# dwipddalal/AttWarp

Measured on AMD Instinct MI355X. Metric: warped images/sec, higher is better.
Workload: dtype f32

## Files before the change

attwarp_amd/csrc/attn_f32v.hpp:

```cpp
#pragma once
#include <type_traits>
#include "common.hpp"

namespace attwarp {

constexpr int ATTN_NT = 256;

struct SharedDiv {
  float d, r1;
  __device__ __forceinline__ explicit SharedDiv(float den) : d(den) {
    const float r0 = __builtin_amdgcn_rcpf(den);
    const float e0 = __builtin_fmaf(-den, r0, 1.0f);
    r1 = __builtin_fmaf(e0, r0, r0);
  }
  __device__ __forceinline__ float operator()(float a) const {
    const float q0 = fmul(a, r1);
    const float e1 = __builtin_fmaf(-d, q0, a);
    const float q1 = __builtin_fmaf(e1, r1, q0);
    const float e2 = __builtin_fmaf(-d, q1, a);
    return __builtin_fmaf(e2, r1, q1);
  }
  __device__ __forceinline__ float first_refinement(float a) const {
    const float q0 = fmul(a, r1);
    const float e1 = __builtin_fmaf(-d, q0, a);
// ... 44 lines not shown
template <typename T> struct Raw4 { uint32_t lo, hi; };
template <> struct Raw4<float> { float x, y, z, w; };
template <typename T> __device__ __forceinline__ Raw4<T> load4_raw(const T* p) {
  typedef uint16_t v4h_a2 __attribute__((ext_vector_type(4), aligned(2)));
  const v4h_a2 q = __builtin_nontemporal_load(reinterpret_cast<const v4h_a2*>(p));
  return Raw4<T>{(uint32_t)q.x | ((uint32_t)q.y << 16), (uint32_t)q.z | ((uint32_t)q.w << 16)};
}
template <> __device__ __forceinline__ Raw4<float> load4_raw<float>(const float* p) {
  const F4v q = load4_nt<float>(p);
  return Raw4<float>{q.x, q.y, q.z, q.w};
}
__device__ __forceinline__ F4v cvt4(const Raw4<float>& r) { return F4v{r.x, r.y, r.z, r.w}; }
__device__ __forceinline__ F4v cvt4(const Raw4<__half>& r) {
  return F4v{__half2float(__builtin_bit_cast(__half, (uint16_t)(r.lo & 0xffffu))), __half2float(__builtin_bit_cast(__half, (uint16_t)(r.lo >> 16))),
             __half2float(__builtin_bit_cast(__half, (uint16_t)(r.hi & 0xffffu))), __half2float(__builtin_bit_cast(__half, (uint16_t)(r.hi >> 16)))};
}
__device__ __forceinline__ F4v cvt4(const Raw4<__hip_bfloat16>& r) {
  return F4v{__uint_as_float(r.lo << 16), __uint_as_float(r.lo & 0xffff0000u), __uint_as_float(r.hi << 16),
             __uint_as_float(r.hi & 0xffff0000u)};
}
template <typename T> __device__ __forceinline__ float round_to(float v) { return to_f32<T>(from_f32<T>(v)); }
template <> __device__ __forceinline__ float round_to<float>(float v) { return v; }

template <typename T>
struct AttnStepArgsT {
  const T* attn;
  int heads;
  int64_t sb, sh, row_off;
  const int32_t* starts;
  int starts_mod, max_start, ntok;
  T* out;
};
typedef AttnStepArgsT<float> AttnStepArgs;
struct AttnStepArgsAny {
  const void* attn;
  int dtype;
  int heads;
  int64_t sb, sh, row_off;
  const int32_t* starts;
  int starts_mod, max_start, ntok;
  void* out;
  template <typename T>
  __device__ __forceinline__ AttnStepArgsT<T> as() const {
    AttnStepArgsT<T> a;
    a.attn = static_cast<const T*>(attn); a.heads = heads; a.sb = sb; a.sh = sh; a.row_off = row_off; a.starts = starts;
    a.starts_mod = starts_mod; a.max_start = max_start; a.ntok = ntok; a.out = static_cast<T*>(out);
    return a;
  }
};
template <int NV>
constexpr size_t attn_v4_lds_bytes() { return (size_t)(ATTN_NT / WAVE) * NV * 4 * WAVE * sizeof(float); }

template <typename T, int NV, int HU>
__device__ __forceinline__ void attn_reduce_v4_block(const AttnStepArgsT<T>& a, int b, float* part) {
  constexpr int NT = ATTN_NT, PW = NV * 4 * WAVE, NW = NT / WAVE;
  const int heads = a.heads, ntok = a.ntok;
  const int64_t sh = a.sh;
  const int lane = threadIdx.x & (WAVE - 1), wid = __builtin_amdgcn_readfirstlane(threadIdx.x / WAVE);
  const int st = min(max(a.starts[b % a.starts_mod], 0), a.max_start);
  const T* base = a.attn + (int64_t)b * a.sb + a.row_off + st;
  float acc[NV][4];
#pragma unroll
  for (int i = 0; i < NV; ++i) acc[i][0] = acc[i][1] = acc[i][2] = acc[i][3] = 0.0f;

  auto head_ptr = [&](int h) { return base + (int64_t)min(h, heads - 1) * sh; };
  const bool tail_room = st + 3 <= a.max_start && ntok < NV * 4 * WAVE;
  auto misalign = [&](const T* rp) { return tail_room ? (int)((reinterpret_cast<uintptr_t>(rp) / sizeof(T)) & 1u) : 0; };
  constexpr bool ALIGN16 = sizeof(T) == 2;
  auto load = [&](Raw4<T> (&r)[HU][NV], int h0) {
#pragma unroll
    for (int u = 0; u < HU; ++u) {
      const T* rp = head_ptr(h0 + u * NW);
      if constexpr (ALIGN16) {
        const int mis = misalign(rp);
        const T* ap = rp - mis;
        const int cmax = (mis + ntok - 1) >> 2;
#pragma unroll
        for (int i = 0; i < NV; ++i) {
          unsigned bo = (unsigned)min(lane + WAVE * i, cmax) * 4u * (unsigned)sizeof(T);
          asm volatile("" : "+v"(bo));
          typedef uint32_t v2u __attribute__((ext_vector_type(2), aligned(2)));
          const v2u q = __builtin_nontemporal_load(reinterpret_cast<const v2u*>(reinterpret_cast<const char*>(ap) + bo));
          r[u][i].lo = q.x;
          r[u][i].hi = q.y;
        }
      } else {
#pragma unroll
        for (int i = 0; i < NV; ++i) {
          const int t = min(4 * lane + 4 * WAVE * i, ntok - 4);
          unsigned bo = (unsigned)t * (unsigned)sizeof(T);
          asm volatile("" : "+v"(bo));
          r[u][i] = load4_raw<T>(reinterpret_cast<const T*>(reinterpret_cast<const char*>(rp) + bo));
        }
      }
    }
  };
  auto next_dword = [&](uint32_t own, uint32_t next_vec) -> uint32_t {
    const uint32_t rot = __builtin_amdgcn_update_dpp(0u, next_vec, 0x134, 0xf, 0xf, false);
    return __builtin_amdgcn_update_dpp(rot, own, 0x130, 0xf, 0xf, false);
  };
  auto realign = [&](const Raw4<T> (&r)[NV], int mis, Raw4<T> (&o)[NV]) {
    if (!ALIGN16 || mis == 0) {
#pragma unroll
      for (int i = 0; i < NV; ++i) o[i] = r[i];
      return;
    }
    if constexpr (ALIGN16) {
#pragma unroll
      for (int i = 0; i < NV; ++i) {
        const Raw4<T>& n = r[i + 1 < NV ? i + 1 : i];
        const uint32_t w2 = next_dword(r[i].lo, n.lo);
        o[i].lo = __builtin_amdgcn_alignbyte(r[i].hi, r[i].lo, 2);
        o[i].hi = __builtin_amdgcn_alignbyte(w2, r[i].hi, 2);
      }
    }
  };
  auto reduce = [&](const Raw4<T> (&r)[HU][NV], int h0) {
#pragma unroll
    for (int u = 0; u < HU; ++u) {
      if (h0 + u * NW < heads) {
        F4v v[NV];
        Raw4<T> sh4[NV];
        realign(r[u], misalign(head_ptr(h0 + u * NW)), sh4);
#pragma unroll
        for (int i = 0; i < NV; ++i) v[i] = cvt4(sh4[i]);
        float s = 0.0f;
#pragma unroll
        for (int i = 0; i < NV; ++i)
          if (4 * lane + 4 * WAVE * i < ntok)
            s = fadd(s, fadd(fadd(v[i].x, v[i].y), fadd(v[i].z, v[i].w)));
        s = wave_sum_dpp(s);
        const float den = to_f32<T>(add_tiny<T>(from_f32<T>(s)));
        constexpr bool kNeedLo = !std::is_same<T, __half>::value;
        uint32_t lo = 0xffffffffu, hi = 0u;
#pragma unroll
        for (int i = 0; i < NV; ++i) {
          const uint32_t bx = __float_as_uint(v[i].x), by = __float_as_uint(v[i].y),
                         bz = __float_as_uint(v[i].z), bw = __float_as_uint(v[i].w);
          if (kNeedLo) lo = min(min(lo, bx - 1u), min(by - 1u, min(bz - 1u, bw - 1u)));
          hi = max(max(hi, bx), max(by, max(bz, bw)));
        }
        const bool box = den >= 8.673617379884035e-19f && den <= 4.0f &&
                         __all(lo >= SDIV_NUM_LO - 1u && hi <= SDIV_NUM_HI);
        if (box) {
          const SharedDiv dv(den);
#pragma unroll
          for (int i = 0; i < NV; ++i) {
            acc[i][0] = fadd(acc[i][0], dv.template rounded_to<T>(v[i].x));
            acc[i][1] = fadd(acc[i][1], dv.template rounded_to<T>(v[i].y));
            acc[i][2] = fadd(acc[i][2], dv.template rounded_to<T>(v[i].z));
            acc[i][3] = fadd(acc[i][3], dv.template rounded_to<T>(v[i].w));
          }
        } else {
#pragma unroll
          for (int i = 0; i < NV; ++i) {
            acc[i][0] = fadd(acc[i][0], round_to<T>(v[i].x / den));
            acc[i][1] = fadd(acc[i][1], round_to<T>(v[i].y / den));
            acc[i][2] = fadd(acc[i][2], round_to<T>(v[i].z / den));
            acc[i][3] = fadd(acc[i][3], round_to<T>(v[i].w / den));
          }
        }
      }
    }
  };
  constexpr int HS = NW * HU;
  for (int h0 = wid; h0 < heads; h0 += HS) {
    Raw4<T> r[HU][NV];
    load(r, h0);
    reduce(r, h0);
  }
#pragma unroll
  for (int i = 0; i < NV; ++i)
#pragma unroll
    for (int j = 0; j < 4; ++j) part[wid * PW + 4 * lane + 4 * WAVE * i + j] = acc[i][j];
  __syncthreads();
  const float nheads = to_f32<T>(from_f32<T>((float)heads));
  for (int t = threadIdx.x; t < ntok; t += NT) {
    float m = 0.0f;
#pragma unroll
    for (int w = 0; w < NW; ++w) m = fadd(m, part[w * PW + t]);
    a.out[(int64_t)b * ntok + t] = from_f32<T>(round_to<T>(m) / nheads);
  }
}


}
```

attwarp_amd/csrc/attn_maps.hip:

```cpp
#include "common.hpp"
#include "axis_blocks.hpp"
#include "attn_f32v.hpp"

#include <algorithm>
#include <cstring>

namespace attwarp {

template <typename T>
__global__ __launch_bounds__(ATTN_NT, 5) void attn_maps_kernel(const AttnStepArgsT<T> a, const StepsMapsArgs m, int n_maps8) {
  extern __shared__ __attribute__((aligned(16))) float am_smem[];
  __shared__ float s_tmp[64], s_pm[64];
  const int blk = blockIdx.x;
  if (blk < n_maps8) {
    if (blk < 2 * m.B) axis_maps_from_steps_block<8, T>(m, blk >> 1, blk & 1, reinterpret_cast<double*>(am_smem), s_tmp, s_pm);
    return;
  }
  attn_reduce_v4_block<T, 3, 4>(a, blk - n_maps8, am_smem);
}

template <typename T>
static int launch_attn_maps(const void* rows, int n_rows, int heads, int kv_len, const int32_t* starts, int starts_mod,
                            int ntok, void* steps_out, const StepsMapsArgs& m, hipStream_t st) {
  AttnStepArgsT<T> a;
  a.attn = static_cast<const T*>(rows); a.heads = heads; a.sb = (int64_t)heads * kv_len; a.sh = kv_len; a.row_off = 0;
  a.starts = starts; a.starts_mod = starts_mod; a.max_start = kv_len - ntok; a.ntok = ntok; a.out = static_cast<T*>(steps_out);
  const int n_maps8 = ((2 * m.B + 7) / 8) * 8;
  const size_t lds = std::max(attn_v4_lds_bytes<3>(), steps_maps_lds_bytes(std::max(m.W, m.H), m.g));
  if (const int rc = grant_dynamic_lds(attn_maps_kernel<T>, lds, "attn_reduce_and_maps")) return rc;
  hipLaunchKernelGGL((attn_maps_kernel<T>), dim3(n_maps8 + n_rows), dim3(ATTN_NT), lds, st, a, m, n_maps8);
  return check_launch("attn_maps_kernel");
}

}

using namespace attwarp;

extern "C" int attwarp_attn_reduce_and_maps(int attn_dtype, const void* rows, int n_rows, int heads, int kv_len,
                                            const int32_t* starts, int starts_mod, int ntok, void* steps_out,
                                            const void* steps_in, int T, int B, int g, int W, int H, int W_out, int H_out,
                                            const double* inv_x, const double* inv_y, float* map_x, float* map_y,
                                            void* stream) {
  ATTWARP_REQUIRE(rows && starts && steps_out && steps_in && inv_x && inv_y && map_x && map_y,
                  "attn_reduce_and_maps: null pointer");
  ATTWARP_REQUIRE(n_rows > 0 && heads > 0 && kv_len > 0 && ntok > 0 && starts_mod > 0 && T > 0 && B > 0 && g > 0 && W > 0 &&
                  H > 0 && W_out > 0 && H_out > 0, "attn_reduce_and_maps: non-positive size");
  ATTWARP_REQUIRE(attn_dtype == ATTWARP_F32 || attn_dtype == ATTWARP_F16 || attn_dtype == ATTWARP_BF16,
                  "attn_reduce_and_maps: attn_dtype must be F32, F16 or BF16 (got %d)", attn_dtype);
  ATTWARP_REQUIRE(ntok <= kv_len, "attn_reduce_and_maps: ntok=%d > kv_len=%d", ntok, kv_len);
  ATTWARP_REQUIRE(steps_out != steps_in, "attn_reduce_and_maps: steps_out must not alias steps_in");
  if (ntok % 4 != 0 || ntok > 3 * 4 * WAVE || ntok != g * g)
    return fail(ATTWARP_E_UNSUPPORTED, "attn_reduce_and_maps: ntok must equal g*g, be a multiple of 4 and <= 768");
  if (g > 32 || std::max(W, H) > 8192 || B > 65535)
    return fail(ATTWARP_E_UNSUPPORTED, "attn_reduce_and_maps: g > 32, max(W,H) > 8192 or B > 65535");
  StepsMapsArgs m;
  m.steps = steps_in; m.step_dtype = attn_dtype; m.T = T; m.B = B; m.g = g; m.W = W; m.H = H; m.W_out = W_out; m.H_out = H_out;
  m.inv_x = inv_x; m.inv_y = inv_y; m.map_x = map_x; m.map_y = map_y; m.att_out = nullptr;
  hipStream_t st = as_stream(stream);
  if (attn_dtype == ATTWARP_F32) return launch_attn_maps<float>(rows, n_rows, heads, kv_len, starts, starts_mod, ntok, steps_out, m, st);
  if (attn_dtype == ATTWARP_F16) return launch_attn_maps<__half>(rows, n_rows, heads, kv_len, starts, starts_mod, ntok, steps_out, m, st);
  return launch_attn_maps<__hip_bfloat16>(rows, n_rows, heads, kv_len, starts, starts_mod, ntok, steps_out, m, st);
}
```

attwarp_amd/csrc/common.hpp:

```cpp
#pragma once
#include <hip/hip_runtime.h>
#include <hip/hip_fp16.h>
#include <hip/hip_bf16.h>
#include <cstdarg>
#include <cstdint>
#include <cstdio>

#include "../../include/attwarp.h"

namespace attwarp {

constexpr int WAVE = 64;

char* error_buffer();
int fail(int code, const char* fmt, ...);

#define ATTWARP_REQUIRE(cond, ...)                                   \
  do {                                                               \
    if (!(cond)) return ::attwarp::fail(ATTWARP_E_ARG, __VA_ARGS__); \
  } while (0)

inline int check_launch(const char* what) {
  hipError_t e = hipGetLastError();
  if (e != hipSuccess) return fail(ATTWARP_E_LAUNCH, "%s: %s", what, hipGetErrorString(e));
  return ATTWARP_OK;
}

__device__ __forceinline__ float fmul(float a, float b) { return __fmul_rn(a, b); }
__device__ __forceinline__ float fadd(float a, float b) { return __fadd_rn(a, b); }
__device__ __forceinline__ float fsub(float a, float b) { return __fsub_rn(a, b); }
__device__ __forceinline__ int cv_round_q5(float m) {
  const float s = fmul(m, 32.0f);
  return (s >= -2147483648.0f && s < 2147483648.0f) ? __float2int_rn(s) : (int)0x80000000;
}
__device__ __forceinline__ float clamp_coord(float m, int size) { return fminf(fmaxf(m, -1.0f), (float)size); }
__device__ __forceinline__ float lerp_rn(float a, float b, float t) { return fadd(a, fmul(t, fsub(b, a))); }

template <typename T>
__device__ __forceinline__ T wave_sum(T v) {
#pragma unroll
  for (int o = WAVE / 2; o > 0; o >>= 1) v += __shfl_xor(v, o, WAVE);
  return v;
}
template <int CTRL, int BANKS>
__device__ __forceinline__ float dpp_f32(float old, float v) {
  return __uint_as_float(__builtin_amdgcn_update_dpp(__float_as_uint(old), __float_as_uint(v), CTRL, 0xf, BANKS, true));
}
__device__ __forceinline__ float wave_sum_dpp(float v) {
  auto a = __builtin_amdgcn_permlane32_swap(__float_as_uint(v), __float_as_uint(v), false, false);
  v = __uint_as_float(a[0]) + __uint_as_float(a[1]);
  auto b = __builtin_amdgcn_permlane16_swap(__float_as_uint(v), __float_as_uint(v), false, false);
  v = __uint_as_float(b[0]) + __uint_as_float(b[1]);
  v = dpp_f32<0x128, 0xf>(0.0f, v) + v;
  float t = dpp_f32<0x104, 0x5>(0.0f, v);
  t = dpp_f32<0x114, 0xa>(t, v);
  v = t + v;
// ... 20 lines not shown
  __syncthreads();
  double t = 0.0;
  for (int i = 0; i < nw; ++i) t += scratch[i];
  return t;
}

template <typename T> __device__ __forceinline__ float to_f32(T v);
template <> __device__ __forceinline__ float to_f32<float>(float v) { return v; }
template <> __device__ __forceinline__ float to_f32<__half>(__half v) { return __half2float(v); }
template <> __device__ __forceinline__ float to_f32<__hip_bfloat16>(__hip_bfloat16 v) { return __bfloat162float(v); }
template <> __device__ __forceinline__ float to_f32<uint8_t>(uint8_t v) { return (float)v; }

template <typename T> __device__ __forceinline__ T from_f32(float v);
template <> __device__ __forceinline__ float from_f32<float>(float v) { return v; }
template <> __device__ __forceinline__ __half from_f32<__half>(float v) { return __float2half_rn(v); }
template <> __device__ __forceinline__ __hip_bfloat16 from_f32<__hip_bfloat16>(float v) { return __float2bfloat16(v); }

template <typename T> __device__ __forceinline__ T from_f64(double v);
template <> __device__ __forceinline__ float from_f64<float>(double v) { return (float)v; }
__device__ __forceinline__ float f64_to_f32_round_odd(double v) {
  float f = (float)v;
  if ((double)f != v) {
    uint32_t u = __float_as_uint(f);
    if (fabs((double)f) > fabs(v)) u -= 1u;
    u |= 1u;
    f = __uint_as_float(u);
  }
  return f;
}
template <> __device__ __forceinline__ __half from_f64<__half>(double v) {
  return __float2half_rn(f64_to_f32_round_odd(v));
}
template <> __device__ __forceinline__ __hip_bfloat16 from_f64<__hip_bfloat16>(double v) {
  return __float2bfloat16(f64_to_f32_round_odd(v));
}

template <typename T> __device__ __forceinline__ T div_t(T a, T b) {
  return from_f32<T>(to_f32<T>(a) / to_f32<T>(b));
}

typedef uint32_t u32_una __attribute__((aligned(1)));

inline hipStream_t as_stream(void* s) { return reinterpret_cast<hipStream_t>(s); }

constexpr size_t LDS_DEFAULT_MAX = 64 * 1024, LDS_CU_BYTES = 160 * 1024;
template <typename K>
inline int grant_dynamic_lds(K kernel, size_t bytes, const char* what, size_t static_bytes = 0) {
  bytes += static_bytes;
  if (bytes <= LDS_DEFAULT_MAX) return ATTWARP_OK;
  if (bytes > LDS_CU_BYTES) return fail(ATTWARP_E_UNSUPPORTED, "%s: needs %zu bytes of LDS (> %zu)", what, bytes, LDS_CU_BYTES);
  const hipError_t e = hipFuncSetAttribute(reinterpret_cast<const void*>(kernel), hipFuncAttributeMaxDynamicSharedMemorySize, (int)bytes);
  if (e != hipSuccess) return fail(ATTWARP_E_UNSUPPORTED, "%s: %zu bytes of dynamic LDS refused: %s", what, bytes, hipGetErrorString(e));
  return ATTWARP_OK;
}

enum TuneKey {
  TUNE_REMAP_VARIANT = 0,
  TUNE_REMAP_ROWS,
  TUNE_REMAP_CHW_SPLIT,
  TUNE_REMAP_TILED,
  TUNE_REMAP_TILE_KO,
  TUNE_REMAP_NOSWZ,
  TUNE_REMAP_NT,
  TUNE_LANCZOS_VARIANT,
  TUNE_CLIP_VARIANT,
  TUNE_PROFILES_VARIANT,
  TUNE_REMAP_CPW,
  TUNE_ATTN_HU,
  TUNE_U8_AHEAD,
  TUNE_TRACE_LO,
  TUNE_TRACE_HI,
  TUNE_PREP_VARIANT,
  TUNE_COUNT
};
#ifdef ATTWARP_TUNING
int tune(TuneKey k);
#else
constexpr int tune(TuneKey) { return -1; }
#endif

#ifdef ATTWARP_TUNING
constexpr int TRACE_WORDS = 16;
inline unsigned long long* trace_buffer() {
  const int lo = tune(TUNE_TRACE_LO), hi = tune(TUNE_TRACE_HI);
  if (lo < 0 || hi < 0) return nullptr;
  return reinterpret_cast<unsigned long long*>(((unsigned long long)hi << 24) | (unsigned long long)lo);
}
#ifdef __HIPCC__
struct TraceStart { unsigned long long real, cyc; };
__device__ __forceinline__ TraceStart trace_now() { return TraceStart{__builtin_amdgcn_s_memrealtime(), __builtin_amdgcn_s_memtime()}; }
__device__ __forceinline__ void trace_mark(unsigned long long* tr, int i) {
  if (tr && threadIdx.x == 0) {
    __builtin_amdgcn_sched_barrier(0);
    unsigned long long* r = tr + TRACE_WORDS * (size_t)blockIdx.x;
    r[6] = 1;
    r[7 + i] = __builtin_amdgcn_s_memtime();
    __builtin_amdgcn_sched_barrier(0);
  }
}
__device__ __forceinline__ void trace_block(unsigned long long* tr, TraceStart t0, int kind) {
  if (!tr) return;
  __syncthreads();
  if (threadIdx.x == 0) {
    unsigned long long* r = tr + TRACE_WORDS * (size_t)blockIdx.x;
    r[0] = t0.real;
    r[1] = __builtin_amdgcn_s_memrealtime();
// ... 12 lines not shown
```

attwarp_amd/csrc/remap_u8.hip:

```cpp
#include "common.hpp"
#include "remap_u8_block.hpp"

namespace attwarp {

namespace u8k {


struct Taps {
  int i0, i1;
  float f;
};
template <int MODE>
__device__ __forceinline__ Taps taps(float m, int size) {
  Taps t;
  int i;
  if (MODE == ATTWARP_CV2) {
    const int q = cv_round_q5(m);
    i = q >> 5;
    t.f = (float)(q & 31);
  } else {
    const float mc = clamp_coord(m, size);
    const float fl = floorf(mc);
    t.f = fsub(mc, fl);
    i = (int)fl;
// ... 219 lines not shown
#undef ATTWARP_U8_ROW
#undef ATTWARP_U8_FLUSH
#undef ATTWARP_U8_FETCH
}

template <int KI, int KO, int MODE>
static int launch_kiko(const Params& p, hipStream_t st) {
  const int VLP = (p.VL + 15) & ~15, OVP = NT * KO;
  const size_t lds = (size_t)(RMAX + 2 * VLP) * sizeof(float) + 2 * (size_t)OVP;
  if (p.NP == 1)
    hipLaunchKernelGGL((remap_rows_u8_kernel<KI, KO, true, false, MODE>), dim3(p.nblocks), dim3(NT), lds, st, p);
  else
    hipLaunchKernelGGL((remap_rows_u8_kernel<KI, KO, false, false, MODE>), dim3(p.nblocks), dim3(NT), lds, st, p);
  return check_launch("remap_rows_u8_kernel");
}

template <int KO, int MODE>
static int launch_ko(const Params& p, hipStream_t st) {
  const int ki = ((p.VL >> 2) + NT - 1) / NT;
  switch (ki) {
    case 1: return launch_kiko<1, KO, MODE>(p, st);
    case 2: return launch_kiko<2, KO, MODE>(p, st);
    case 3: return launch_kiko<3, KO, MODE>(p, st);
    default: return launch_kiko<4, KO, MODE>(p, st);
  }
}

template <int KI, int KD, bool HWC, int PD, bool UA>
__global__ __launch_bounds__(NT) void remap_rows_u8i_kernel(const Params p) {
  extern __shared__ __attribute__((aligned(16))) float smem[];
  remap_rows_u8i_block<KI, KD, HWC, PD, UA>(p, blockIdx.x, smem);
}

template <int KI, int PD>
static int launch_u8i_ki(const Params& p, hipStream_t st) {
  const size_t lds = (size_t)RMAX * sizeof(float) + 2 * (size_t)U8I_VLP * sizeof(uint16_t);
  const int kd = ((((p.OVL + 3) >> 2)) + NT - 1) / NT;
  const dim3 g(p.nblocks), t(NT);
#define ATTWARP_U8I_LAUNCH(KD)                                                                              \
  if (p.unaligned) hipLaunchKernelGGL((remap_rows_u8i_kernel<KI, KD, true, PD, true>), g, t, lds, st, p);    \
  else if (p.NP == 1) hipLaunchKernelGGL((remap_rows_u8i_kernel<KI, KD, true, PD, false>), g, t, lds, st, p); \
  else hipLaunchKernelGGL((remap_rows_u8i_kernel<KI, KD, false, PD, false>), g, t, lds, st, p)
  if (kd <= 1) { ATTWARP_U8I_LAUNCH(1); } else if (kd == 2) { ATTWARP_U8I_LAUNCH(2); }
  else if (kd == 3) { ATTWARP_U8I_LAUNCH(3); } else { ATTWARP_U8I_LAUNCH(4); }
#undef ATTWARP_U8I_LAUNCH
  return check_launch("remap_rows_u8i_kernel");
}
template <int KI>
static int launch_u8i_depth(const Params& p, hipStream_t st) {
#ifdef ATTWARP_TUNING
  if (tune(TUNE_U8_AHEAD) == 1) return launch_u8i_ki<KI, 1>(p, st);
  if (tune(TUNE_U8_AHEAD) == 2) return launch_u8i_ki<KI, 2>(p, st);
  if (tune(TUNE_U8_AHEAD) == 4) return launch_u8i_ki<KI, 4>(p, st);
#endif
  return launch_u8i_ki<KI, (KI <= 2 ? 4 : 2)>(p, st);
}
static int launch_u8i(const Params& p, hipStream_t st) {
  const int ki = (((p.VL + 3) >> 2) + NT - 1) / NT;
  switch (ki) {
    case 1: return launch_u8i_depth<1>(p, st);
    case 2: return launch_u8i_depth<2>(p, st);
    case 3: return launch_u8i_depth<3>(p, st);
    default: return launch_u8i_depth<4>(p, st);
  }
}

template <int MODE>
static int launch_mode(const Params& p, bool tiled, hipStream_t st) {
  constexpr int TILE_KO = 8, TILE_KI = 3;
  if (tiled) {
    const size_t lds = (size_t)(RMAX + 2 * TILE_KI * NT * 4) * sizeof(float) + 2 * (size_t)(NT * TILE_KO);
    hipLaunchKernelGGL((remap_rows_u8_kernel<TILE_KI, TILE_KO, true, true, MODE>), dim3(p.nblocks), dim3(NT), lds, st, p);
    return check_launch("remap_rows_u8_kernel");
  }
  const int ko = (p.OVL + NT - 1) / NT;
  if (ko <= 4) return launch_ko<4, MODE>(p, st);
  if (ko <= 8) return launch_ko<8, MODE>(p, st);
  if (ko <= 12) return launch_ko<12, MODE>(p, st);
  return launch_ko<16, MODE>(p, st);
}

}

static bool plan_u8(u8k::Params& p, const uint8_t* src, uint8_t* dst, int layout, int B, int C, int H, int W, int Ho, int Wo,
                    const float* mx, const float* my, int mode, bool* tiled_out, bool* integer_out) {
  if (tune(TUNE_REMAP_VARIANT) == 1) return false;
  p.src = src; p.dst = dst; p.mx = mx; p.my = my;
  p.H = H; p.W = W; p.Ho = Ho; p.Wo = Wo;
  if (layout == ATTWARP_HWC) { p.NP = 1; p.CS = C; } else { p.NP = C; p.CS = 1; }
  p.row_len = W * p.CS;
  p.orow_len = Wo * p.CS;
  long long VL = (long long)p.NP * p.row_len, OVL = (long long)p.NP * p.orow_len;
  bool ua = p.row_len % 4 != 0 || p.orow_len % 4 != 0 ||
            ((reinterpret_cast<uintptr_t>(src) | reinterpret_cast<uintptr_t>(dst)) & 3u) != 0 ||
            (layout == ATTWARP_HWC ? ((long long)H * W * C) % 4 != 0 || ((long long)Ho * Wo * C) % 4 != 0
                                   : ((long long)H * W) % 4 != 0 || ((long long)Ho * Wo) % 4 != 0);
  if (ua && (mode != ATTWARP_CV2 || tune(TUNE_REMAP_VARIANT) == 2)) return false;
  p.map_div = 1;
  p.ntiles = 1;
  p.grp = tune(TUNE_REMAP_NOSWZ) >= 0 ? tune(TUNE_REMAP_NOSWZ) : 0;
  bool tiled = VL > 4096 || OVL > 4096;
  if (ua && layout != ATTWARP_HWC && p.row_len <= 4096 && p.orow_len <= 4096) tiled = false;
  if (ua && (tiled || p.row_len < 4)) return false;
  if (tiled || (ua && layout != ATTWARP_HWC)) {
    if (tiled && tune(TUNE_REMAP_TILED) == 0) return false;
    if ((long long)p.row_len > 2147483647LL / 8 || (long long)p.orow_len > 2147483647LL / 8 ||
// ... 69 lines not shown
```

attwarp_amd/csrc/remap_u8_block.hpp:

```cpp
#pragma once
#include "common.hpp"

namespace attwarp {
namespace u8k {

constexpr int NT = 256;
constexpr int RMAX = 64;

struct Params {
  const uint8_t* src;
  uint8_t* dst;
  const float* mx;
  const float* my;
  int H, W, Ho, Wo;
  int NP, CS;
  int row_len, orow_len;
  int VL, OVL;
  long long img_stride, plane_stride, oimg_stride, oplane_stride;
  int R, nblk, nblocks;
  int wpi;
  int grp;
  int ntiles;
  int map_div;
  int unaligned;
};

constexpr int U8I_STORE_NT = 2;
constexpr int U8I_VLP = 4096 + 16;

constexpr size_t u8i_lds_bytes() { return (size_t)RMAX * sizeof(float) + 2 * (size_t)U8I_VLP * sizeof(uint16_t); }
template <int KI, int KD, bool HWC, int PD, bool UA>
__device__ __forceinline__ void remap_rows_u8i_rows(const Params& p, const uint8_t* src_b, int img_bytes, uint8_t* dst_b,
                                                    int oimg_bytes, const float* mx_b, const float* my_b, int rb0, float* smem) {
  static_assert(!UA || HWC, "unaligned rows: interleaved images only (planar ones are dispatched plane by plane)");
  float* s_my = smem;
  uint16_t* vrow0 = reinterpret_cast<uint16_t*>(smem + RMAX);
  uint16_t* vrow1 = vrow0 + U8I_VLP;
  const int tid = threadIdx.x;
  const unsigned base_sh = UA ? (unsigned)(reinterpret_cast<uintptr_t>(src_b) & 3u) : 0u;
  const __amdgpu_buffer_rsrc_t rsrc = __builtin_amdgcn_make_buffer_rsrc(
      const_cast<uint8_t*>(src_b) - base_sh, 0, UA ? (int)((img_bytes + base_sh + 3u) & ~3u) : img_bytes, 0x00020000);
  const __amdgpu_buffer_rsrc_t rdst = __builtin_amdgcn_make_buffer_rsrc(dst_b, 0, oimg_bytes, 0x00020000);

  unsigned goff[KI];
  int voff[KI];
  {
    const int dpr = p.row_len >> 2, nd = UA ? (p.VL + 3) >> 2 : p.VL >> 2;
#pragma unroll
    for (int k = 0; k < KI; ++k) {
      const int d = min(tid + NT * k, nd - 1);
      const int pl = HWC ? 0 : d / dpr;
      goff[k] = (unsigned)(pl * p.plane_stride) + 4u * (unsigned)(d - pl * dpr);
      voff[k] = 4 * d;
    }
  }
  unsigned t0[KD][4], t1[KD][4], wpk[KD][4];
  int soff[KD];
  {
    const int dpo = p.orow_len >> 2, ndo = UA ? (p.OVL + 3) >> 2 : p.OVL >> 2;
    const unsigned vbase = (unsigned)(uintptr_t)(__attribute__((address_space(3))) uint16_t*)vrow0;
    auto lds_off = [vbase](unsigned e) -> unsigned { return vbase + 2u * ((e & ~3u) | (((e & 1u) << 1) | ((e >> 1) & 1u))); };
#pragma unroll
    for (int k = 0; k < KD; ++k) {
      const int d = min(tid + NT * k, ndo - 1);
      const int pl = HWC ? 0 : d / dpo;
      const int r0 = 4 * (d - pl * dpo);
      soff[k] = (int)(pl * p.oplane_stride) + r0;
      int xj = r0 / p.CS, cj = r0 - xj * p.CS;
#pragma unroll
      for (int j = 0; j < 4; ++j) {
        const int x = UA ? min(xj, p.Wo - 1) : xj, c = cj;
        if (++cj >= p.CS) { cj = 0; ++xj; }
        const float m = mx_b[x];
        const int q = cv_round_q5(m);
        const int i = q >> 5;
        const int i0 = min(max(i, 0), p.W - 1), i1 = min(max(i + 1, 0), p.W - 1);
        const unsigned kx = (i0 == i1) ? 0u : (unsigned)(q & 31);
        const unsigned e0 = (unsigned)(pl * p.row_len + i0 * p.CS + c);
        const unsigned e1 = (i0 == i1) ? e0 : (unsigned)(pl * p.row_len + i1 * p.CS + c);
        t0[k][j] = lds_off(e0);
        t1[k][j] = lds_off(e1);
        asm volatile("" : "+v"(t0[k][j]), "+v"(t1[k][j]));
        wpk[k][j] = ((32u - kx) << 6) | (kx << 22);
      }
    }
  }

  typedef unsigned short us2 __attribute__((ext_vector_type(2)));
  typedef __attribute__((address_space(3))) const uint16_t lds_cu16;
  auto row_taps = [&](float m, int& i0, int& i1, unsigned& ky) {
    const int q = cv_round_q5(m);
    const int i = q >> 5;
    i0 = min(max(i, 0), p.H - 1);
    i1 = min(max(i + 1, 0), p.H - 1);
    ky = (unsigned)(q & 31);
  };
  int ci0, ci1;
  unsigned ky[PD];
  uint32_t A[PD][KI], C[PD][KI];
  uint32_t A1[PD][UA ? KI : 1], C1[PD][UA ? KI : 1];
  unsigned sha[PD], shc[PD];
  int y0 = 0, nrows = 0;
#define ATTWARP_U8I_FETCH(AX, CX, AX1, CX1, SA, SC)                                                    \
  {                                                                                                    \
    int ra_ = ci0 * p.row_len, rc_ = ci1 * p.row_len;                          \
    if (UA) {                                                                                          \
      ra_ += (int)base_sh; rc_ += (int)base_sh;                                                        \
      SA = (unsigned)ra_ & 3u; SC = (unsigned)rc_ & 3u;                                                \
      ra_ &= ~3; rc_ &= ~3;                                                                            \
    }                                                                                                  \
    _Pragma("unroll") for (int k = 0; k < KI; ++k) {                                                    \
      AX[k] = __builtin_amdgcn_raw_buffer_load_b32(rsrc, (int)goff[k], ra_, 0);                         \
      CX[k] = __builtin_amdgcn_raw_buffer_load_b32(rsrc, (int)goff[k], rc_, 0);                         \
       \
      if (UA && SA) AX1[k] = __builtin_amdgcn_raw_buffer_load_b32(rsrc, (int)goff[k] + 4, ra_, 0);      \
      if (UA && SC) CX1[k] = __builtin_amdgcn_raw_buffer_load_b32(rsrc, (int)goff[k] + 4, rc_, 0);      \
    }                                                                                                  \
  }
#define ATTWARP_U8I_ROW(q_, vbuf, VOFF, AX, CX, KY, AX1, CX1, SA, SC)                                  \
  {                                                                                                    \
    const unsigned w1_ = KY, w0_ = 32u - KY;                                                           \
    if (UA) {                       \
      _Pragma("unroll") for (int k = 0; k < KI; ++k) {                                                  \
        AX[k] = __builtin_amdgcn_alignbyte(AX1[k], AX[k], SA);                                         \
        CX[k] = __builtin_amdgcn_alignbyte(CX1[k], CX[k], SC);                                         \
      }                                                                                                \
    }                                                                                                  \
    const us2 w0p_ = {(unsigned short)w0_, (unsigned short)w0_}, w1p_ = {(unsigned short)w1_, (unsigned short)w1_}; \
    _Pragma("unroll") for (int k = 0; k < KI; ++k) {                                                    \
       \
      const uint32_t a02_ = AX[k] & 0x00ff00ffu, a13_ = __builtin_amdgcn_perm(0u, AX[k], 0x0c030c01u);   \
      const uint32_t c02_ = CX[k] & 0x00ff00ffu, c13_ = __builtin_amdgcn_perm(0u, CX[k], 0x0c030c01u);   \
      const us2 v02_ = __builtin_bit_cast(us2, a02_) * w0p_ + __builtin_bit_cast(us2, c02_) * w1p_;      \
      const us2 v13_ = __builtin_bit_cast(us2, a13_) * w0p_ + __builtin_bit_cast(us2, c13_) * w1p_;      \
      uint2 st_;                                                                                       \
      st_.x = __builtin_bit_cast(uint32_t, v02_);                                                      \
      st_.y = __builtin_bit_cast(uint32_t, v13_);                                                      \
      *reinterpret_cast<uint2*>((vbuf) + voff[k]) = st_;                                               \
    }                                                                                                  \
    if ((q_) + PD < nrows) {    \
      row_taps(s_my[(q_) + PD], ci0, ci1, KY);                                                         \
      ATTWARP_U8I_FETCH(AX, CX, AX1, CX1, SA, SC)                                                      \
    }                                                                                                  \
    __syncthreads();                                                                                   \
    const int orow_ = (y0 + (q_)) * p.orow_len;                                                        \
    _Pragma("unroll") for (int k = 0; k < KD; ++k) {                                                    \
      unsigned v0_[4], v1_[4];                                                                         \
      _Pragma("unroll") for (int j = 0; j < 4; ++j) {                                                   \
        v0_[j] = *(lds_cu16*)(uintptr_t)(t0[k][j] + (VOFF));                                           \
        v1_[j] = *(lds_cu16*)(uintptr_t)(t1[k][j] + (VOFF));                                           \
      }                                                                                                \
                                                   \
      unsigned r_[4];                                                                                  \
      _Pragma("unroll") for (int j = 0; j < 4; ++j) {                                                   \
        const us2 pr_ = {(unsigned short)v0_[j], (unsigned short)v1_[j]};                               \
        r_[j] = __builtin_amdgcn_udot2(pr_, __builtin_bit_cast(us2, wpk[k][j]), 512u << 6, false);      \
      }                                                                                                \
      const unsigned o_ = __builtin_amdgcn_perm(r_[1], r_[0], 0x0c0c0602u) | __builtin_amdgcn_perm(r_[3], r_[2], 0x06020c0cu); \
      if (tid + NT * k < (p.OVL >> 2)) __builtin_amdgcn_raw_buffer_store_b32(o_, rdst, soff[k], orow_, U8I_STORE_NT); \
      else if (UA && k == KD - 1 && tid + NT * k == (p.OVL >> 2)) {              \
        for (int j_ = 0; j_ < (p.OVL & 3); ++j_)                                                       \
          __builtin_amdgcn_raw_buffer_store_b8((uint8_t)(o_ >> (8 * j_)), rdst, soff[k] + j_, orow_, U8I_STORE_NT); \
      }                                                                                                \
    }                                                                                                  \
  }
  for (int rb = rb0; rb < p.nblk; rb += p.wpi) {
    y0 = rb * p.R;
    nrows = min(y0 + p.R, p.Ho) - y0;
    if (rb != rb0) __syncthreads();
    if (tid < nrows) s_my[tid] = my_b[y0 + tid];
    __syncthreads();
#pragma unroll
    for (int u = 0; u < PD; ++u)
      if (u < nrows) {
        row_taps(s_my[u], ci0, ci1, ky[u]);
        ATTWARP_U8I_FETCH(A[u], C[u], A1[u], C1[u], sha[u], shc[u])
      }
    int q = 0;
    for (; q + 3 < nrows; q += 4) {
      ATTWARP_U8I_ROW(q, vrow0, 0u, A[0], C[0], ky[0], A1[0], C1[0], sha[0], shc[0])
      ATTWARP_U8I_ROW(q + 1, vrow1, 2u * U8I_VLP, A[1 % PD], C[1 % PD], ky[1 % PD], A1[1 % PD], C1[1 % PD], sha[1 % PD], shc[1 % PD])
      ATTWARP_U8I_ROW(q + 2, vrow0, 0u, A[2 % PD], C[2 % PD], ky[2 % PD], A1[2 % PD], C1[2 % PD], sha[2 % PD], shc[2 % PD])
      ATTWARP_U8I_ROW(q + 3, vrow1, 2u * U8I_VLP, A[3 % PD], C[3 % PD], ky[3 % PD], A1[3 % PD], C1[3 % PD], sha[3 % PD], shc[3 % PD])
    }
    if (q < nrows) ATTWARP_U8I_ROW(q, vrow0, 0u, A[0], C[0], ky[0], A1[0], C1[0], sha[0], shc[0])
    if (q + 1 < nrows) ATTWARP_U8I_ROW(q + 1, vrow1, 2u * U8I_VLP, A[1 % PD], C[1 % PD], ky[1 % PD], A1[1 % PD], C1[1 % PD], sha[1 % PD], shc[1 % PD])
    if (q + 2 < nrows) ATTWARP_U8I_ROW(q + 2, vrow0, 0u, A[2 % PD], C[2 % PD], ky[2 % PD], A1[2 % PD], C1[2 % PD], sha[2 % PD], shc[2 % PD])
  }
#undef ATTWARP_U8I_ROW
#undef ATTWARP_U8I_FETCH
}

template <int KI, int KD, bool HWC, int PD, bool UA = false>
__device__ __forceinline__ void remap_rows_u8i_block(const Params& p, int bid_in, float* smem) {
  int bid = bid_in;
  {
    const int n = p.nblocks, q = n >> 3, r = n & 7, xcd = bid & 7, idx = bid >> 3;
    if (p.grp == 0) bid = (xcd < r) ? xcd * (q + 1) + idx : r * (q + 1) + (xcd - r) * q + idx;
    else if (p.grp >= 2) {
      const int g = p.grp, per = 8 * g, grp = idx / g, within = idx - grp * g, cand = grp * per + xcd * g + within;
      bid = cand < (n / per) * per ? cand : bid;
    }
  }
  const int b = bid / p.wpi, rb0 = bid - b * p.wpi, bm = b / p.map_div;
  remap_rows_u8i_rows<KI, KD, HWC, PD, UA>(p, p.src + (long long)b * p.img_stride, (int)p.img_stride,
                                           p.dst + (long long)b * p.oimg_stride, (int)p.oimg_stride,
                                           p.mx + (long long)bm * p.Wo, p.my + (long long)bm * p.Ho, rb0, smem);
}

}

bool u8i_params(u8k::Params& p, const uint8_t* src, uint8_t* dst, int layout, int B, int C, int H, int W, int Ho, int Wo,
                const float* mx, const float* my);

}
```

Measured before the change: 218,700.

## Make attention reduce persistent with cross-row prefetch of head loads

Replaces the one-block-per-row attention reduction with a persistent grid sized to CU count times occupancy. Each workgroup walks rows with a stride and software-pipelines its loads: the next head group, and the first heads of the next row, are issued before the current reduce or epilogue runs. Start offsets are read through scalar constant-address loads. This aims to hide global-load latency and cut block launch/tail overhead, at the cost of an extra barrier per row and more live registers.

```diff
diff --git a/attwarp_amd/csrc/attn_f32v.hpp b/attwarp_amd/csrc/attn_f32v.hpp
--- a/attwarp_amd/csrc/attn_f32v.hpp
+++ b/attwarp_amd/csrc/attn_f32v.hpp
@@ -120,22 +120,38 @@
 constexpr size_t attn_v4_lds_bytes() { return (size_t)(ATTN_NT / WAVE) * NV * 4 * WAVE * sizeof(float); }
 
 template <typename T, int NV, int HU>
-__device__ __forceinline__ void attn_reduce_v4_block(const AttnStepArgsT<T>& a, int b, float* part) {
-  constexpr int NT = ATTN_NT, PW = NV * 4 * WAVE, NW = NT / WAVE;
-  const int heads = a.heads, ntok = a.ntok;
-  const int64_t sh = a.sh;
-  const int lane = threadIdx.x & (WAVE - 1), wid = __builtin_amdgcn_readfirstlane(threadIdx.x / WAVE);
-  const int st = min(max(a.starts[b % a.starts_mod], 0), a.max_start);
-  const T* base = a.attn + (int64_t)b * a.sb + a.row_off + st;
+struct AttnReduceV4 {
+  static constexpr int NT = ATTN_NT, PW = NV * 4 * WAVE, NW = NT / WAVE;
+  static constexpr int HS = NW * HU;
+  static constexpr bool ALIGN16 = sizeof(T) == 2;
+  const AttnStepArgsT<T>& a;
+  const int heads, ntok;
+  const int64_t sh;
+  const int lane, wid;
+  const T* base;
+  bool tail_room;
   float acc[NV][4];
-#pragma unroll
-  for (int i = 0; i < NV; ++i) acc[i][0] = acc[i][1] = acc[i][2] = acc[i][3] = 0.0f;
-
-  auto head_ptr = [&](int h) { return base + (int64_t)min(h, heads - 1) * sh; };
-  const bool tail_room = st + 3 <= a.max_start && ntok < NV * 4 * WAVE;
-  auto misalign = [&](const T* rp) { return tail_room ? (int)((reinterpret_cast<uintptr_t>(rp) / sizeof(T)) & 1u) : 0; };
-  constexpr bool ALIGN16 = sizeof(T) == 2;
-  auto load = [&](Raw4<T> (&r)[HU][NV], int h0) {
+
+  __device__ __forceinline__ explicit AttnReduceV4(const AttnStepArgsT<T>& args)
+      : a(args), heads(args.heads), ntok(args.ntok), sh(args.sh), lane(threadIdx.x & (WAVE - 1)),
+        wid(__builtin_amdgcn_readfirstlane(threadIdx.x / WAVE)), base(nullptr), tail_room(false) {
+    clear();
+  }
+  __device__ __forceinline__ void clear() {
+#pragma unroll
+    for (int i = 0; i < NV; ++i) acc[i][0] = acc[i][1] = acc[i][2] = acc[i][3] = 0.0f;
+  }
+  __device__ __forceinline__ void sample(int b, int start) {
+    const int st = min(max(start, 0), a.max_start);
+    base = a.attn + (int64_t)b * a.sb + a.row_off + st;
+    tail_room = st + 3 <= a.max_start && ntok < NV * 4 * WAVE;
+  }
+
+  __device__ __forceinline__ const T* head_ptr(int h) const { return base + (int64_t)min(h, heads - 1) * sh; }
+  __device__ __forceinline__ int misalign(const T* rp) const {
+    return tail_room ? (int)((reinterpret_cast<uintptr_t>(rp) / sizeof(T)) & 1u) : 0;
+  }
+  __device__ __forceinline__ void load(Raw4<T> (&r)[HU][NV], int h0) const {
 #pragma unroll
     for (int u = 0; u < HU; ++u) {
       const T* rp = head_ptr(h0 + u * NW);
@@ -162,12 +178,12 @@
         }
       }
     }
-  };
-  auto next_dword = [&](uint32_t own, uint32_t next_vec) -> uint32_t {
+  }
+  static __device__ __forceinline__ uint32_t next_dword(uint32_t own, uint32_t next_vec) {
     const uint32_t rot = __builtin_amdgcn_update_dpp(0u, next_vec, 0x134, 0xf, 0xf, false);
     return __builtin_amdgcn_update_dpp(rot, own, 0x130, 0xf, 0xf, false);
-  };
-  auto realign = [&](const Raw4<T> (&r)[NV], int mis, Raw4<T> (&o)[NV]) {
+  }
+  static __device__ __forceinline__ void realign(const Raw4<T> (&r)[NV], int mis, Raw4<T> (&o)[NV]) {
     if (!ALIGN16 || mis == 0) {
 #pragma unroll
       for (int i = 0; i < NV; ++i) o[i] = r[i];
@@ -182,8 +198,8 @@
         o[i].hi = __builtin_amdgcn_alignbyte(w2, r[i].hi, 2);
       }
     }
-  };
-  auto reduce = [&](const Raw4<T> (&r)[HU][NV], int h0) {
+  }
+  __device__ __forceinline__ void reduce(const Raw4<T> (&r)[HU][NV], int h0) {
 #pragma unroll
     for (int u = 0; u < HU; ++u) {
       if (h0 + u * NW < heads) {
@@ -230,26 +246,72 @@
         }
       }
     }
-  };
-  constexpr int HS = NW * HU;
-  for (int h0 = wid; h0 < heads; h0 += HS) {
+  }
+  __device__ __forceinline__ void epilogue(int b, float* part) const {
+#pragma unroll
+    for (int i = 0; i < NV; ++i)
+#pragma unroll
+      for (int j = 0; j < 4; ++j) part[wid * PW + 4 * lane + 4 * WAVE * i + j] = acc[i][j];
+    __syncthreads();
+    const float nheads = to_f32<T>(from_f32<T>((float)heads));
+    for (int t = threadIdx.x; t < ntok; t += NT) {
+      float m = 0.0f;
+#pragma unroll
+      for (int w = 0; w < NW; ++w) m = fadd(m, part[w * PW + t]);
+      a.out[(int64_t)b * ntok + t] = from_f32<T>(round_to<T>(m) / nheads);
+    }
+  }
+};
+
+template <typename T, int NV, int HU>
+__device__ __forceinline__ void attn_reduce_v4_block(const AttnStepArgsT<T>& a, int b, float* part) {
+  AttnReduceV4<T, NV, HU> blk(a);
+  blk.sample(b, a.starts[b % a.starts_mod]);
+  for (int h0 = blk.wid; h0 < blk.heads; h0 += blk.HS) {
     Raw4<T> r[HU][NV];
-    load(r, h0);
-    reduce(r, h0);
-  }
-#pragma unroll
-  for (int i = 0; i < NV; ++i)
-#pragma unroll
-    for (int j = 0; j < 4; ++j) part[wid * PW + 4 * lane + 4 * WAVE * i + j] = acc[i][j];
-  __syncthreads();
-  const float nheads = to_f32<T>(from_f32<T>((float)heads));
-  for (int t = threadIdx.x; t < ntok; t += NT) {
-    float m = 0.0f;
-#pragma unroll
-    for (int w = 0; w < NW; ++w) m = fadd(m, part[w * PW + t]);
-    a.out[(int64_t)b * ntok + t] = from_f32<T>(round_to<T>(m) / nheads);
-  }
-}
-
-
-}
+    blk.load(r, h0);
+    blk.reduce(r, h0);
+  }
+  blk.epilogue(b, part);
+}
+
+__device__ __forceinline__ int32_t load_uniform_const(const int32_t* p) {
+  return *(const __attribute__((address_space(4))) int32_t*)p;
+}
+template <typename T, int NV, int HU>
+__device__ __forceinline__ void attn_reduce_v4_walk(const AttnStepArgsT<T>& a, int w, int nwg, int n_rows, float* part) {
+  AttnReduceV4<T, NV, HU> blk(a);
+  const int mod = a.starts_mod, stride = nwg % mod;
+  auto advance = [&](int si) { si += stride; return si >= mod ? si - mod : si; };
+  int n = w, si = n % mod;
+  int start = load_uniform_const(a.starts + si);
+  si = advance(si);
+  int start_next = n + nwg < n_rows ? load_uniform_const(a.starts + si) : 0;
+  Raw4<T> r[HU][NV];
+  blk.sample(n, start);
+  if (blk.wid < blk.heads) blk.load(r, blk.wid);
+  for (;;) {
+    for (int h0 = blk.wid; h0 < blk.heads;) {
+      blk.reduce(r, h0);
+      h0 += blk.HS;
+      if (h0 < blk.heads) blk.load(r, h0);
+    }
+    const int nn = n + nwg;
+    const bool more = nn < n_rows;
+    if (more) {
+      blk.sample(nn, start_next);
+      if (blk.wid < blk.heads) blk.load(r, blk.wid);
+      si = advance(si);
+      if (nn + nwg < n_rows) start_next = load_uniform_const(a.starts + si);
+    }
+    __builtin_amdgcn_sched_barrier(0);
+    blk.epilogue(n, part);
+    if (!more) break;
+    n = nn;
+    blk.clear();
+    __syncthreads();
+  }
+}
+
+
+}
diff --git a/attwarp_amd/csrc/attn_maps.hip b/attwarp_amd/csrc/attn_maps.hip
--- a/attwarp_amd/csrc/attn_maps.hip
+++ b/attwarp_amd/csrc/attn_maps.hip
@@ -7,8 +7,10 @@
 
 namespace attwarp {
 
+constexpr int ATTN_WALK_WG_PER_CU = 5;
 template <typename T>
-__global__ __launch_bounds__(ATTN_NT, 5) void attn_maps_kernel(const AttnStepArgsT<T> a, const StepsMapsArgs m, int n_maps8) {
+__global__ __launch_bounds__(ATTN_NT, ATTN_WALK_WG_PER_CU) void attn_maps_kernel(const AttnStepArgsT<T> a, const StepsMapsArgs m, int n_maps8,
+                                                                                 int n_walk, int n_rows) {
   extern __shared__ __attribute__((aligned(16))) float am_smem[];
   __shared__ float s_tmp[64], s_pm[64];
   const int blk = blockIdx.x;
@@ -16,7 +18,7 @@
     if (blk < 2 * m.B) axis_maps_from_steps_block<8, T>(m, blk >> 1, blk & 1, reinterpret_cast<double*>(am_smem), s_tmp, s_pm);
     return;
   }
-  attn_reduce_v4_block<T, 3, 4>(a, blk - n_maps8, am_smem);
+  attn_reduce_v4_walk<T, 3, 4>(a, blk - n_maps8, n_walk, n_rows, am_smem);
 }
 
 template <typename T>
@@ -26,9 +28,13 @@
   a.attn = static_cast<const T*>(rows); a.heads = heads; a.sb = (int64_t)heads * kv_len; a.sh = kv_len; a.row_off = 0;
   a.starts = starts; a.starts_mod = starts_mod; a.max_start = kv_len - ntok; a.ntok = ntok; a.out = static_cast<T*>(steps_out);
   const int n_maps8 = ((2 * m.B + 7) / 8) * 8;
+  const int cus = device_cu_count();
+  if (cus <= 0) return ATTWARP_E_LAUNCH;
+  const int64_t slots = (int64_t)ATTN_WALK_WG_PER_CU * cus;
+  const int n_walk = (int)std::min<int64_t>(n_rows, n_maps8 <= slots - cus ? slots - n_maps8 : slots);
   const size_t lds = std::max(attn_v4_lds_bytes<3>(), steps_maps_lds_bytes(std::max(m.W, m.H), m.g));
   if (const int rc = grant_dynamic_lds(attn_maps_kernel<T>, lds, "attn_reduce_and_maps")) return rc;
-  hipLaunchKernelGGL((attn_maps_kernel<T>), dim3(n_maps8 + n_rows), dim3(ATTN_NT), lds, st, a, m, n_maps8);
+  hipLaunchKernelGGL((attn_maps_kernel<T>), dim3(n_maps8 + n_walk), dim3(ATTN_NT), lds, st, a, m, n_maps8, n_walk, n_rows);
   return check_launch("attn_maps_kernel");
 }
 
diff --git a/attwarp_amd/csrc/common.hpp b/attwarp_amd/csrc/common.hpp
--- a/attwarp_amd/csrc/common.hpp
+++ b/attwarp_amd/csrc/common.hpp
@@ -2,6 +2,7 @@
 #include <hip/hip_runtime.h>
 #include <hip/hip_fp16.h>
 #include <hip/hip_bf16.h>
+#include <atomic>
 #include <cstdarg>
 #include <cstdint>
 #include <cstdio>
@@ -128,6 +129,25 @@
   const hipError_t e = hipFuncSetAttribute(reinterpret_cast<const void*>(kernel), hipFuncAttributeMaxDynamicSharedMemorySize, (int)bytes);
   if (e != hipSuccess) return fail(ATTWARP_E_UNSUPPORTED, "%s: %zu bytes of dynamic LDS refused: %s", what, bytes, hipGetErrorString(e));
   return ATTWARP_OK;
+}
+
+inline int device_cu_count() {
+  constexpr int MAX_DEV = 64;
+  static std::atomic<int> cached[MAX_DEV];
+  int dev = 0;
+  hipError_t e = hipGetDevice(&dev);
+  if (e == hipSuccess && dev >= 0 && dev < MAX_DEV) {
+    const int have = cached[dev].load(std::memory_order_relaxed);
+    if (have > 0) return have;
+  }
+  int cus = 0;
+  if (e == hipSuccess) e = hipDeviceGetAttribute(&cus, hipDeviceAttributeMultiprocessorCount, dev);
+  if (e != hipSuccess || cus <= 0) {
+    fail(ATTWARP_E_LAUNCH, "device_cu_count: %s", e != hipSuccess ? hipGetErrorString(e) : "no compute units reported");
+    return 0;
+  }
+  if (dev >= 0 && dev < MAX_DEV) cached[dev].store(cus, std::memory_order_relaxed);
+  return cus;
 }
 
 enum TuneKey {
```

Result: no change. 218,600 (median of 2 runs) (-0.0%).

## Make u8 row-pipeline branch-free with null-range buffer ops and prefetched row maps

Applied to the files above, without the earlier changes.

Removes the data-dependent branches around prefetch loads and stores in the interleaved u8 remap pipeline. Out-of-range work is now masked through buffer resources with zero record count, or an out-of-bounds store offset, so the buffer hardware drops it. In unaligned mode both spill words are always loaded. The next row-block's y-map value is prefetched into a register before the barrier, and an unroll factor that is a multiple of both the prefetch depth and the double-buffer count is added, along with depths 3 and 8 as tuning options and a scheduling barrier per row. The goal is a uniform instruction stream with less scalar branching and exposed latency. The cost is extra dummy memory instructions, including null stores in the prologue, and higher register use.

```diff
diff --git a/attwarp_amd/csrc/remap_u8.hip b/attwarp_amd/csrc/remap_u8.hip
--- a/attwarp_amd/csrc/remap_u8.hip
+++ b/attwarp_amd/csrc/remap_u8.hip
@@ -295,6 +295,8 @@
   if (tune(TUNE_U8_AHEAD) == 1) return launch_u8i_ki<KI, 1>(p, st);
   if (tune(TUNE_U8_AHEAD) == 2) return launch_u8i_ki<KI, 2>(p, st);
   if (tune(TUNE_U8_AHEAD) == 4) return launch_u8i_ki<KI, 4>(p, st);
+  if (tune(TUNE_U8_AHEAD) == 3) return launch_u8i_ki<KI, 3>(p, st);
+  if (tune(TUNE_U8_AHEAD) == 8) return launch_u8i_ki<KI, 8>(p, st);
 #endif
   return launch_u8i_ki<KI, (KI <= 2 ? 4 : 2)>(p, st);
 }
diff --git a/attwarp_amd/csrc/remap_u8_block.hpp b/attwarp_amd/csrc/remap_u8_block.hpp
--- a/attwarp_amd/csrc/remap_u8_block.hpp
+++ b/attwarp_amd/csrc/remap_u8_block.hpp
@@ -38,8 +38,6 @@
   uint16_t* vrow1 = vrow0 + U8I_VLP;
   const int tid = threadIdx.x;
   const unsigned base_sh = UA ? (unsigned)(reinterpret_cast<uintptr_t>(src_b) & 3u) : 0u;
-  const __amdgpu_buffer_rsrc_t rsrc = __builtin_amdgcn_make_buffer_rsrc(
-      const_cast<uint8_t*>(src_b) - base_sh, 0, UA ? (int)((img_bytes + base_sh + 3u) & ~3u) : img_bytes, 0x00020000);
   const __amdgpu_buffer_rsrc_t rdst = __builtin_amdgcn_make_buffer_rsrc(dst_b, 0, oimg_bytes, 0x00020000);
 
   unsigned goff[KI];
@@ -65,7 +63,7 @@
       const int d = min(tid + NT * k, ndo - 1);
       const int pl = HWC ? 0 : d / dpo;
       const int r0 = 4 * (d - pl * dpo);
-      soff[k] = (int)(pl * p.oplane_stride) + r0;
+      soff[k] = (tid + NT * k < (p.OVL >> 2)) ? (int)(pl * p.oplane_stride) + r0 : (int)0x80000000u;
       int xj = r0 / p.CS, cj = r0 - xj * p.CS;
 #pragma unroll
       for (int j = 0; j < 4; ++j) {
@@ -101,7 +99,9 @@
   uint32_t A1[PD][UA ? KI : 1], C1[PD][UA ? KI : 1];
   unsigned sha[PD], shc[PD];
   int y0 = 0, nrows = 0;
-#define ATTWARP_U8I_FETCH(AX, CX, AX1, CX1, SA, SC)                                                    \
+  const int src_records = UA ? (int)((img_bytes + base_sh + 3u) & ~3u) : img_bytes;
+  const __amdgpu_buffer_rsrc_t rdst_none = __builtin_amdgcn_make_buffer_rsrc(dst_b, 0, 0, 0x00020000);
+#define ATTWARP_U8I_FETCH(AX, CX, AX1, CX1, SA, SC, LIVE)                                              \
   {                                                                                                    \
     int ra_ = ci0 * p.row_len, rc_ = ci1 * p.row_len;                          \
     if (UA) {                                                                                          \
@@ -109,12 +109,16 @@
       SA = (unsigned)ra_ & 3u; SC = (unsigned)rc_ & 3u;                                                \
       ra_ &= ~3; rc_ &= ~3;                                                                            \
     }                                                                                                  \
+    const __amdgpu_buffer_rsrc_t rs_ = __builtin_amdgcn_make_buffer_rsrc(                              \
+        const_cast<uint8_t*>(src_b) - base_sh, 0, (LIVE) ? src_records : 0, 0x00020000);               \
     _Pragma("unroll") for (int k = 0; k < KI; ++k) {                                                    \
-      AX[k] = __builtin_amdgcn_raw_buffer_load_b32(rsrc, (int)goff[k], ra_, 0);                         \
-      CX[k] = __builtin_amdgcn_raw_buffer_load_b32(rsrc, (int)goff[k], rc_, 0);                         \
+      AX[k] = __builtin_amdgcn_raw_buffer_load_b32(rs_, (int)goff[k], ra_, 0);                          \
+      CX[k] = __builtin_amdgcn_raw_buffer_load_b32(rs_, (int)goff[k], rc_, 0);                          \
        \
-      if (UA && SA) AX1[k] = __builtin_amdgcn_raw_buffer_load_b32(rsrc, (int)goff[k] + 4, ra_, 0);      \
-      if (UA && SC) CX1[k] = __builtin_amdgcn_raw_buffer_load_b32(rsrc, (int)goff[k] + 4, rc_, 0);      \
+      if (UA) {                                                                                        \
+        AX1[k] = __builtin_amdgcn_raw_buffer_load_b32(rs_, (int)goff[k] + 4, ra_, 0);                   \
+        CX1[k] = __builtin_amdgcn_raw_buffer_load_b32(rs_, (int)goff[k] + 4, rc_, 0);                   \
+      }                                                                                                \
     }                                                                                                  \
   }
 #define ATTWARP_U8I_ROW(q_, vbuf, VOFF, AX, CX, KY, AX1, CX1, SA, SC)                                  \
@@ -138,9 +142,9 @@
       st_.y = __builtin_bit_cast(uint32_t, v13_);                                                      \
       *reinterpret_cast<uint2*>((vbuf) + voff[k]) = st_;                                               \
     }                                                                                                  \
-    if ((q_) + PD < nrows) {    \
-      row_taps(s_my[(q_) + PD], ci0, ci1, KY);                                                         \
-      ATTWARP_U8I_FETCH(AX, CX, AX1, CX1, SA, SC)                                                      \
+    {  \
+      row_taps(s_my[min((q_) + PD, nrows - 1)], ci0, ci1, KY);                                         \
+      ATTWARP_U8I_FETCH(AX, CX, AX1, CX1, SA, SC, (q_) + PD < nrows)                                   \
     }                                                                                                  \
     __syncthreads();                                                                                   \
     const int orow_ = (y0 + (q_)) * p.orow_len;                                                        \
@@ -157,36 +161,63 @@
         r_[j] = __builtin_amdgcn_udot2(pr_, __builtin_bit_cast(us2, wpk[k][j]), 512u << 6, false);      \
       }                                                                                                \
       const unsigned o_ = __builtin_amdgcn_perm(r_[1], r_[0], 0x0c0c0602u) | __builtin_amdgcn_perm(r_[3], r_[2], 0x06020c0cu); \
-      if (tid + NT * k < (p.OVL >> 2)) __builtin_amdgcn_raw_buffer_store_b32(o_, rdst, soff[k], orow_, U8I_STORE_NT); \
-      else if (UA && k == KD - 1 && tid + NT * k == (p.OVL >> 2)) {              \
+      __builtin_amdgcn_raw_buffer_store_b32(o_, rdst, soff[k], orow_, U8I_STORE_NT);    \
+      if (UA && k == KD - 1 && tid + NT * k == (p.OVL >> 2)) {                   \
         for (int j_ = 0; j_ < (p.OVL & 3); ++j_)                                                       \
-          __builtin_amdgcn_raw_buffer_store_b8((uint8_t)(o_ >> (8 * j_)), rdst, soff[k] + j_, orow_, U8I_STORE_NT); \
-      }                                                                                                \
-    }                                                                                                  \
-  }
+          __builtin_amdgcn_raw_buffer_store_b8((uint8_t)(o_ >> (8 * j_)), rdst, (p.OVL & ~3) + j_, orow_, U8I_STORE_NT); \
+      }                                                                                                \
+    }                                                                                                  \
+    __builtin_amdgcn_sched_barrier(0);                                                                 \
+  }
+#define ATTWARP_U8I_ROWU(u)                                                                            \
+  ATTWARP_U8I_ROW(q + (u), ((u) & 1) ? vrow1 : vrow0, ((u) & 1) ? 2u * U8I_VLP : 0u, A[(u) % PD], C[(u) % PD], ky[(u) % PD], \
+                  A1[(u) % PD], C1[(u) % PD], sha[(u) % PD], shc[(u) % PD])
+  constexpr int U = (PD == 3) ? 6 : (PD == 8) ? 8 : 4;
+  static_assert(U % PD == 0 && U % 2 == 0, "register set and LDS buffer of a row must be compile-time");
+  float my_next = my_b[min(rb0 * p.R + tid, p.Ho - 1)];
   for (int rb = rb0; rb < p.nblk; rb += p.wpi) {
     y0 = rb * p.R;
     nrows = min(y0 + p.R, p.Ho) - y0;
     if (rb != rb0) __syncthreads();
-    if (tid < nrows) s_my[tid] = my_b[y0 + tid];
+    if (tid < nrows) s_my[tid] = my_next;
+    my_next = my_b[min((rb + p.wpi) * p.R + tid, p.Ho - 1)];
     __syncthreads();
 #pragma unroll
-    for (int u = 0; u < PD; ++u)
-      if (u < nrows) {
-        row_taps(s_my[u], ci0, ci1, ky[u]);
-        ATTWARP_U8I_FETCH(A[u], C[u], A1[u], C1[u], sha[u], shc[u])
+    for (int u = 0; u < PD; ++u) {
+      row_taps(s_my[min(u, nrows - 1)], ci0, ci1, ky[u]);
+      ATTWARP_U8I_FETCH(A[u], C[u], A1[u], C1[u], sha[u], shc[u], u < nrows)
+#pragma unroll
+      for (int k = 0; k < KD; ++k)
+        __builtin_amdgcn_raw_buffer_store_b32(0u, rdst_none, soff[k], 4 * (u * KD + k), U8I_STORE_NT);
+    }
+    int q = 0;
+    for (; q + U - 1 < nrows; q += U) {
+      ATTWARP_U8I_ROWU(0) ATTWARP_U8I_ROWU(1) ATTWARP_U8I_ROWU(2) ATTWARP_U8I_ROWU(3)
+      if constexpr (U > 4) { ATTWARP_U8I_ROWU(4) ATTWARP_U8I_ROWU(5) }
+      if constexpr (U > 6) { ATTWARP_U8I_ROWU(6) ATTWARP_U8I_ROWU(7) }
+    }
+    do {
+      if (q >= nrows) break;
+      ATTWARP_U8I_ROWU(0)
+      if (q + 1 >= nrows) break;
+      ATTWARP_U8I_ROWU(1)
+      if (q + 2 >= nrows) break;
+      ATTWARP_U8I_ROWU(2)
+      if constexpr (U > 4) {
+        if (q + 3 >= nrows) break;
+        ATTWARP_U8I_ROWU(3)
+        if (q + 4 >= nrows) break;
+        ATTWARP_U8I_ROWU(4)
       }
-    int q = 0;
-    for (; q + 3 < nrows; q += 4) {
-      ATTWARP_U8I_ROW(q, vrow0, 0u, A[0], C[0], ky[0], A1[0], C1[0], sha[0], shc[0])
-      ATTWARP_U8I_ROW(q + 1, vrow1, 2u * U8I_VLP, A[1 % PD], C[1 % PD], ky[1 % PD], A1[1 % PD], C1[1 % PD], sha[1 % PD], shc[1 % PD])
-      ATTWARP_U8I_ROW(q + 2, vrow0, 0u, A[2 % PD], C[2 % PD], ky[2 % PD], A1[2 % PD], C1[2 % PD], sha[2 % PD], shc[2 % PD])
-      ATTWARP_U8I_ROW(q + 3, vrow1, 2u * U8I_VLP, A[3 % PD], C[3 % PD], ky[3 % PD], A1[3 % PD], C1[3 % PD], sha[3 % PD], shc[3 % PD])
-    }
-    if (q < nrows) ATTWARP_U8I_ROW(q, vrow0, 0u, A[0], C[0], ky[0], A1[0], C1[0], sha[0], shc[0])
-    if (q + 1 < nrows) ATTWARP_U8I_ROW(q + 1, vrow1, 2u * U8I_VLP, A[1 % PD], C[1 % PD], ky[1 % PD], A1[1 % PD], C1[1 % PD], sha[1 % PD], shc[1 % PD])
-    if (q + 2 < nrows) ATTWARP_U8I_ROW(q + 2, vrow0, 0u, A[2 % PD], C[2 % PD], ky[2 % PD], A1[2 % PD], C1[2 % PD], sha[2 % PD], shc[2 % PD])
-  }
+      if constexpr (U > 6) {
+        if (q + 5 >= nrows) break;
+        ATTWARP_U8I_ROWU(5)
+        if (q + 6 >= nrows) break;
+        ATTWARP_U8I_ROWU(6)
+      }
+    } while (false);
+  }
+#undef ATTWARP_U8I_ROWU
 #undef ATTWARP_U8I_ROW
 #undef ATTWARP_U8I_FETCH
 }
```

New measurement: 214,300 before, 213,900 after. No clear change (-0.2%).
